# huggingface/distil-whisper

Hardware: AMD Instinct MI355X
Metric: training audio-seconds/s (distil-large-v3 student, 30 s clips) (higher is better)
Workload: dtype bf16

## Files before the change

### distil_whisper_amd/csrc/attention.hip

```cpp
#include "common.h"
#include "../../include/dwamd.h"

#define NEG_BIG (-1.0e30f)
#ifndef DW_ATTN_DEFER
#define DW_ATTN_DEFER 8
#endif
#ifndef DW_ATTN_IDLE_SKIP
#define DW_ATTN_IDLE_SKIP 1
#endif
typedef __attribute__((ext_vector_type(4))) unsigned u32x4;

struct AttnP {
    const bf16* q; const bf16* k; const bf16* v; bf16* o; float* lse;
    const bf16* d_o; float* delta; bf16* dq; bf16* dk; bf16* dv;
    long ldq, ldk, ldv, ldo, lddo, lddq, lddk, lddv;
    int B, H, Lq, Lk;
    long q_rows, kv_rows;
    float* dq_colsum;
    float* dv_colsum;
    const int* q_start; const int* q_len;
    const int* kv_start; const int* kv_len;
    int kv_B;
    int plain_order;
    float defer;
// ... 37 lines not shown
    char* const wr = patch + ln * 144 + hi * 8;
#pragma unroll
    for (int cb = 0; cb < 2; ++cb) {
        const f32x16& a = cb == 0 ? a0 : a1;
#pragma unroll
        for (int g = 0; g < 4; ++g) {
            bf16x4 w;
#pragma unroll
            for (int e = 0; e < 4; ++e) w[e] = f2bf(a[g * 4 + e] * mul);
            *(bf16x4*)(wr + cb * 64 + g * 16) = w;
        }
    }
    const int rr = lane >> 3, sc = lane & 7;
    u32x4 o[4];
#pragma unroll
    for (int it = 0; it < 4; ++it) o[it] = *(const u32x4*)(patch + (it * 8 + rr) * 144 + sc * 16);
    const unsigned loff = (unsigned)(rr * (int)ld + sc * 8) * 2u;
    char* const rb = (char*)(base + (long)row0 * ld);
#pragma unroll
    for (int it = 0; it < 4; ++it)
        if (row0 + it * 8 + rr < nrows) *(u32x4*)(rb + (long)it * 8 * ld * 2 + loff) = o[it];
}

__device__ __forceinline__ void colsum_t(float* colsum, bool ok, int cb, int hi, int ln, const f32x16& a, float mul) {
#pragma unroll
    for (int r = 0; r < 16; ++r) {
        float v = ok ? bf2f(f2bf(a[r] * mul)) : 0.f;
#pragma unroll
        for (int o = 1; o < 32; o <<= 1) v += __shfl_xor(v, o);
        if (ln == 0) atomicAdd(colsum + cb * 32 + (r & 3) + 8 * (r >> 2) + 4 * hi, v);
    }
}

__device__ __forceinline__ void attn_workgroup(int ntile, int H, bool plain, int& tile, int& h, int& b) {
    const int n = gridDim.x, L = blockIdx.x;
    const int xcd = L & 7, slot = L >> 3, q = n >> 3, r = n & 7;
    const int logical = plain ? L : xcd * q + min(xcd, r) + slot;
    tile = logical % ntile;
    const int bh = logical / ntile;
    h = bh % H;
    b = bh / H;
}

template <bool CAUSAL, int NW = 4, int ABL = 0, bool VL = false>
__global__ __launch_bounds__(64 * NW, CAUSAL ? 2 : 4) void attn_fwd_kernel(const AttnP p) {
    __shared__ __attribute__((aligned(1024))) char smem[2 * 16384];
    const int lane = threadIdx.x & 63;
    const int wave = __builtin_amdgcn_readfirstlane(threadIdx.x >> 6);
    const int hi = lane >> 5, ln = lane & 31;
    int tile, h, b;
    attn_workgroup((p.Lq + 32 * NW - 1) / (32 * NW), p.H, p.plain_order, tile, h, b);
    const int qb0 = tile * (32 * NW);
    long q_row0 = (long)b * p.q_rows, kv_row0 = (long)b * p.kv_rows;
    int Lq = p.Lq, Lk = p.Lk;
    if constexpr (VL) {
        q_row0 = p.q_start[b];
        Lq = p.q_len[b];
        if (p.kv_start) { kv_row0 = p.kv_start[b]; Lk = p.kv_len[b]; }
        else kv_row0 = (long)min(b, p.kv_B - 1) * p.kv_rows;
        if (qb0 >= Lq) return;
    }
    const int q = qb0 + wave * 32 + ln;
    const bool q_ok = q < Lq;
    const int qc = q_ok ? q : Lq - 1;
    const bf16* Q = p.q + q_row0 * p.ldq + h * 64;
    const bf16* K = p.k + kv_row0 * p.ldk + h * 64;
    const bf16* V = p.v + kv_row0 * p.ldv + h * 64;

    bf16x8 qf[4];
#pragma unroll
    for (int kk = 0; kk < 4; ++kk) qf[kk] = ldg8(Q, qc, p.ldq, kk * 16 + hi * 8);

    int nkt = (Lk + 63) >> 6;
    if (CAUSAL) {
        const int lim = ((min(qb0 + 32 * NW - 1, Lq - 1) + p.coff) >> 6) + 1;
        nkt = min(nkt, lim);
    }
    const float c = p.scale * 1.4426950408889634f;
    float m_run = NEG_BIG, l_run = 0.f;
    f32x16 o[2];
#pragma unroll
    for (int r = 0; r < 16; ++r) { o[0][r] = 0.f; o[1][r] = 0.f; }

    stage_tile64<NW>(K, p.ldk, 0, Lk, smem, wave, lane);
    stage_tile64<NW>(V, p.ldv, 0, Lk, smem + 8192, wave, lane);
    for (int kt = 0; kt < nkt; ++kt) {
        const int buf = kt & 1;
        if (!(ABL & 16) || kt == 0) {
            wait_vm0_seen();
            __syncthreads();
        }
        if (kt + 1 < nkt && !(ABL & 8)) {
            stage_tile64<NW>(K, p.ldk, (kt + 1) * 64, Lk, smem + (buf ^ 1) * 16384, wave, lane);
            stage_tile64<NW>(V, p.ldv, (kt + 1) * 64, Lk, smem + (buf ^ 1) * 16384 + 8192, wave, lane);
        }
        const char* tK = smem + buf * 16384;
        const char* tV = tK + 8192;
        if (DW_ATTN_IDLE_SKIP && qb0 + wave * 32 >= Lq) continue;
        f32x16 s[2];
#pragma unroll
        for (int kb = 0; kb < 2; ++kb) {
#pragma unroll
            for (int r = 0; r < 16; ++r) s[kb][r] = (ABL & 32) ? o[kb][r] : 0.f;
            if (!(ABL & 32)) {
#pragma unroll
                for (int kk = 0; kk < 4; ++kk)
                    s[kb] = __builtin_amdgcn_mfma_f32_32x32x16_bf16((ABL & 2) ? qf[kk ^ kb] : frag_rows(tK, kb, kk, lane), qf[kk], s[kb], 0, 0, 0);
            }
        }
        const int wq0 = qb0 + wave * 32 + (CAUSAL ? p.coff : 0);
        const bool need_mask = ((kt + 1) * 64 > Lk) || (CAUSAL && kt * 64 + 63 > wq0);
        if (CAUSAL && kt * 64 > wq0 + 31) continue;
        float mx = NEG_BIG;
        if (need_mask) {
#pragma unroll
            for (int kb = 0; kb < 2; ++kb)
#pragma unroll
                for (int r = 0; r < 16; ++r) {
                    const int key = kt * 64 + kb * 32 + (r & 3) + 8 * (r >> 2) + 4 * hi;
                    const bool ok = key < Lk && (!CAUSAL || key <= q + p.coff);
                    s[kb][r] = ok ? s[kb][r] : NEG_BIG;
                }
        }
#pragma unroll
        for (int kb = 0; kb < 2; ++kb)
#pragma unroll
            for (int r = 0; r < 16; ++r) mx = fmaxf(mx, s[kb][r]);
        mx = xhalf_max(mx);
        const bool move = __any((mx - m_run) * c > p.defer);
        const float m_new = move ? fmaxf(m_run, mx) : m_run;
        const float mc = m_new * c;
        f32x2 rs2[2] = {{0.f, 0.f}, {0.f, 0.f}};
        const f32x2 c2 = {c, c}, mc2 = {mc, mc};
#pragma unroll
        for (int kb = 0; kb < 2; ++kb)
#pragma unroll
            for (int r = 0; r < 16; r += 2) {
                f32x2 t = {s[kb][r], s[kb][r + 1]};
                t = t * c2 - mc2;
                f32x2 pv = {__builtin_amdgcn_exp2f(t[0]), __builtin_amdgcn_exp2f(t[1])};
                if (ABL & 1) pv = t;
                s[kb][r] = pv[0];
                s[kb][r + 1] = pv[1];
                rs2[(r >> 1) & 1] += pv;
            }
        rs2[0] += rs2[1];
        float rs = rs2[0][0] + rs2[0][1];
        rs = xhalf_sum(rs);
        if (move) {
            const float alpha = __builtin_amdgcn_exp2f((m_run - m_new) * c);
            l_run *= alpha;
#pragma unroll
            for (int r = 0; r < 16; ++r) { o[0][r] *= alpha; o[1][r] *= alpha; }
        }
        l_run += rs;
        m_run = m_new;
#pragma unroll
        for (int kb = 0; kb < 2; ++kb)
#pragma unroll
            for (int s2 = 0; s2 < 2; ++s2) {
                const bf16x8 pf = pack8(s[kb], s2);
                const int rb = kb * 32 + s2 * 16 + hi * 4;
                if (ABL & 64) {
                    o[kb][s2] += bf2f(pf[0]) + bf2f(pf[2]) + bf2f(pf[4]) + bf2f(pf[6]);
                    continue;
                }
#pragma unroll
                for (int db = 0; db < 2; ++db)
                    o[db] = __builtin_amdgcn_mfma_f32_32x32x16_bf16((ABL & 4) ? qf[db * 2 + s2] : frag_tr(tV, db, rb, rb + 8, lane), pf, o[db], 0, 0, 0);
            }
    }
    const float inv = 1.0f / l_run;
    bf16* O = p.o + q_row0 * p.ldo + h * 64;
    if (DW_ATTN_ROWSTORE && NW <= 7 && (p.ldo & 7) == 0 && ((uintptr_t)p.o & 15) == 0) {
        __syncthreads();
        store_rows(O, p.ldo, qb0 + wave * 32, Lq, smem + wave * 4608, lane, o[0], o[1], inv);
    } else {
        store_t(O, p.ldo, q, q_ok, 0, hi, o[0], inv);
        store_t(O, p.ldo, q, q_ok, 1, hi, o[1], inv);
    }
    if (!VL && p.lse && q_ok && hi == 0) p.lse[((long)b * p.H + h) * Lq + q] = m_run * p.scale + __logf(l_run);
}

template <int NW = 4, int OCC = 3>
__global__ __launch_bounds__(64 * NW, OCC) void attn_fwd_pipe_kernel(const AttnP p) {
    __shared__ __attribute__((aligned(1024))) char smem[3 * 16384];
    const int lane = threadIdx.x & 63;
    const int wave = __builtin_amdgcn_readfirstlane(threadIdx.x >> 6);
    const int hi = lane >> 5, ln = lane & 31;
    int tile, h, b;
    attn_workgroup((p.Lq + 32 * NW - 1) / (32 * NW), p.H, p.plain_order, tile, h, b);
    const int qb0 = tile * (32 * NW);
    const int q = qb0 + wave * 32 + ln;
    const bool q_ok = q < p.Lq;
    const int qc = q_ok ? q : p.Lq - 1;
    const bf16* Q = p.q + (long)b * p.q_rows * p.ldq + h * 64;
    const bf16* K = p.k + (long)b * p.kv_rows * p.ldk + h * 64;
    const bf16* V = p.v + (long)b * p.kv_rows * p.ldv + h * 64;
    bf16x8 qf[4];
#pragma unroll
    for (int kk = 0; kk < 4; ++kk) qf[kk] = ldg8(Q, qc, p.ldq, kk * 16 + hi * 8);
    const int nkt = (p.Lk + 63) >> 6;
    const float c = p.scale * 1.4426950408889634f;
    float m_run = NEG_BIG, l_run = 0.f;
    f32x16 o[2];
#pragma unroll
    for (int r = 0; r < 16; ++r) { o[0][r] = 0.f; o[1][r] = 0.f; }

    auto stage = [&](int kt, int st) __attribute__((always_inline)) {
        stage_tile64<NW>(K, p.ldk, kt * 64, p.Lk, smem + st * 16384, wave, lane);
        stage_tile64<NW>(V, p.ldv, kt * 64, p.Lk, smem + st * 16384 + 8192, wave, lane);
    };
    auto scores = [&](int kt, int st, f32x16 (&s)[2]) __attribute__((always_inline)) {
        const char* tK = smem + st * 16384;
#pragma unroll
        for (int kb = 0; kb < 2; ++kb) {
#pragma unroll
            for (int r = 0; r < 16; ++r) s[kb][r] = 0.f;
#pragma unroll
            for (int kk = 0; kk < 4; ++kk)
                s[kb] = __builtin_amdgcn_mfma_f32_32x32x16_bf16(frag_rows(tK, kb, kk, lane), qf[kk], s[kb], 0, 0, 0);
        }
        if ((kt + 1) * 64 > p.Lk) {
#pragma unroll
            for (int kb = 0; kb < 2; ++kb)
#pragma unroll
                for (int r = 0; r < 16; ++r) {
                    const int key = kt * 64 + kb * 32 + (r & 3) + 8 * (r >> 2) + 4 * hi;
                    s[kb][r] = key < p.Lk ? s[kb][r] : NEG_BIG;
                }
        }
    };
    auto softmax_pv = [&](int st, f32x16 (&s)[2]) __attribute__((always_inline)) {
        const char* tV = smem + st * 16384 + 8192;
        float mx = NEG_BIG;
#pragma unroll
        for (int kb = 0; kb < 2; ++kb)
#pragma unroll
            for (int r = 0; r < 16; ++r) mx = fmaxf(mx, s[kb][r]);
        mx = xhalf_max(mx);
        const bool move = __any((mx - m_run) * c > p.defer);
        const float m_new = move ? fmaxf(m_run, mx) : m_run;
        const float mc = m_new * c;
        f32x2 rs2[2] = {{0.f, 0.f}, {0.f, 0.f}};
        const f32x2 c2 = {c, c}, mc2 = {mc, mc};
#pragma unroll
        for (int kb = 0; kb < 2; ++kb)
#pragma unroll
            for (int r = 0; r < 16; r += 2) {
                f32x2 t = {s[kb][r], s[kb][r + 1]};
                t = t * c2 - mc2;
                const f32x2 pv = {__builtin_amdgcn_exp2f(t[0]), __builtin_amdgcn_exp2f(t[1])};
                s[kb][r] = pv[0];
                s[kb][r + 1] = pv[1];
                rs2[(r >> 1) & 1] += pv;
            }
        rs2[0] += rs2[1];
        float rs = rs2[0][0] + rs2[0][1];
        rs = xhalf_sum(rs);
        if (move) {
            const float alpha = __builtin_amdgcn_exp2f((m_run - m_new) * c);
            l_run *= alpha;
#pragma unroll
            for (int r = 0; r < 16; ++r) { o[0][r] *= alpha; o[1][r] *= alpha; }
        }
        l_run += rs;
        m_run = m_new;
#pragma unroll
        for (int kb = 0; kb < 2; ++kb)
#pragma unroll
            for (int s2 = 0; s2 < 2; ++s2) {
                const bf16x8 pf = pack8(s[kb], s2);
                const int rb = kb * 32 + s2 * 16 + hi * 4;
#pragma unroll
                for (int db = 0; db < 2; ++db)
                    o[db] = __builtin_amdgcn_mfma_f32_32x32x16_bf16(frag_tr(tV, db, rb, rb + 8, lane), pf, o[db], 0, 0, 0);
            }
    };

    stage(0, 0);
    if (nkt > 1) stage(1, 1);
    wait_vm0_seen();
    __syncthreads();
    f32x16 sa[2], sb[2];
    scores(0, 0, sa);
    auto iter = [&](int kt, int st0, int st1, int st2, f32x16 (&cur)[2], f32x16 (&nxt)[2]) __attribute__((always_inline)) {
        if (kt > 0) {
            wait_vm0_seen();
            __syncthreads();
        }
        if (kt + 2 < nkt) stage(kt + 2, st2);
        if (kt + 1 < nkt) scores(kt + 1, st1, nxt);
        softmax_pv(st0, cur);
    };
    int st0 = 0, st1 = 1, st2 = 2;
    for (int kt = 0; kt < nkt; kt += 2) {
        iter(kt, st0, st1, st2, sa, sb);
        if (kt + 1 < nkt) iter(kt + 1, st1, st2, st0, sb, sa);
        const int t0 = st0; st0 = st2; st2 = st1; st1 = t0;
    }
    const float inv = 1.0f / l_run;
    bf16* O = p.o + (long)b * p.q_rows * p.ldo + h * 64;
    if (DW_ATTN_ROWSTORE && (p.ldo & 7) == 0 && ((uintptr_t)p.o & 15) == 0) {
        __syncthreads();
        store_rows(O, p.ldo, qb0 + wave * 32, p.Lq, smem + wave * 4608, lane, o[0], o[1], inv);
    } else {
        store_t(O, p.ldo, q, q_ok, 0, hi, o[0], inv);
        store_t(O, p.ldo, q, q_ok, 1, hi, o[1], inv);
    }
    if (p.lse && q_ok && hi == 0) p.lse[((long)b * p.H + h) * p.Lq + q] = m_run * p.scale + __logf(l_run);
}

template <int NW, bool PRE>
__global__ __launch_bounds__(64 * NW) void attn_decode_kernel(const AttnP p) {
    extern __shared__ __attribute__((aligned(16))) float dsm[];
    const int lane = threadIdx.x & 63;
    const int wave = __builtin_amdgcn_readfirstlane(threadIdx.x >> 6);
    const int h = blockIdx.y, b = blockIdx.z;
    const int sub = lane >> 3, ds = (lane & 7) * 8;
    float* sc = dsm;
    float* part = dsm + ((p.Lk + 3) & ~3);
    float* redm = part + NW * 64;
    float* redl = redm + NW;
    const bf16* Q = p.q + (long)b * p.q_rows * p.ldq + h * 64 + ds;
    const bf16* K = p.k + (long)b * p.kv_rows * p.ldk + h * 64 + ds;
    const bf16* V = p.v + (long)b * p.kv_rows * p.ldv + h * 64 + ds;
    const float c = p.scale * 1.4426950408889634f;
    float qv[8];
    {
        const bf16x8 q8 = *(const bf16x8*)Q;
#pragma unroll
        for (int e = 0; e < 8; ++e) qv[e] = bf2f(q8[e]) * c;
    }
    constexpr int NIT = 12;
    bf16x8 kr[PRE ? NIT : 1], vr[PRE ? NIT : 1];
    if constexpr (PRE) {
#pragma unroll
        for (int it = 0; it < NIT; ++it) {
            int k = wave * 8 + it * (NW * 8) + sub;
            k = k < p.Lk ? k : p.Lk - 1;
            kr[it] = ld_stream<2>((const bf16x8*)(K + (long)k * p.ldk));
        }
#pragma unroll
        for (int it = 0; it < NIT; ++it) {
            int k = wave * 8 + it * (NW * 8) + sub;
            k = k < p.Lk ? k : p.Lk - 1;
            vr[it] = ld_stream<2>((const bf16x8*)(V + (long)k * p.ldv));
        }
    }
    float mx = NEG_BIG;
    float sreg[PRE ? NIT : 1];
    if constexpr (PRE) {
#pragma unroll
        for (int it = 0; it < NIT; ++it) {
            const int k = wave * 8 + it * (NW * 8) + sub;
            float s = 0.f;
#pragma unroll
            for (int e = 0; e < 8; ++e) s = fmaf(qv[e], bf2f(kr[it][e]), s);
            s += __shfl_xor(s, 1);
            s += __shfl_xor(s, 2);
            s += __shfl_xor(s, 4);
            sreg[it] = s;
            if (k < p.Lk) mx = fmaxf(mx, s);
        }
    } else {
    for (int k0 = wave * 8; k0 < p.Lk; k0 += NW * 8) {
        const int k = k0 + sub;
        float s = 0.f;
        if (k < p.Lk) {
            const bf16x8 k8 = *(const bf16x8*)(K + (long)k * p.ldk);
#pragma unroll
            for (int e = 0; e < 8; ++e) s = fmaf(qv[e], bf2f(k8[e]), s);
        }
        s += __shfl_xor(s, 1);
        s += __shfl_xor(s, 2);
        s += __shfl_xor(s, 4);
        if (k < p.Lk) {
            if ((lane & 7) == 0) sc[k] = s;
            mx = fmaxf(mx, s);
        }
    }
    }
    mx = wave_max(mx);
    if (lane == 0) redm[wave] = mx;
    __syncthreads();
    mx = redm[0];
#pragma unroll
    for (int i = 1; i < NW; ++i) mx = fmaxf(mx, redm[i]);
    float o[8] = {0.f, 0.f, 0.f, 0.f, 0.f, 0.f, 0.f, 0.f};
    float l = 0.f;
    if constexpr (PRE) {
#pragma unroll
        for (int it = 0; it < NIT; ++it) {
// ... 240 lines not shown
        const char* tG = tQ + 8192;
        const float* tL = (const float*)(tQ + 16384);
        const float* tD = tL + 64;
        const bool need_mask = MODE == 1 || (MODE == 2 && (((qt + 1) * 64 > p.Lq) || (wk0 + 31 >= p.Lk) || (CAUSAL && wk0 + 31 > qt * 64)));
        if (CAUSAL && wk0 > qt * 64 + 63) continue;
        if (DW_ATTN_IDLE_SKIP && wk0 >= p.Lk) continue;
#pragma unroll
        for (int qb = 0; qb < 2; ++qb) {
            f32x16 s, dp;
#pragma unroll
            for (int g = 0; g < 4; ++g) {
                const int ql = qb * 32 + g * 8 + hi * 4;
                const f32x4 l4 = *(const f32x4*)(tL + ql);
                const f32x4 d4 = *(const f32x4*)(tD + ql);
#pragma unroll
                for (int e = 0; e < 4; ++e) { s[g * 4 + e] = l4[e]; dp[g * 4 + e] = d4[e]; }
            }
#pragma unroll
            for (int kk = 0; kk < 4; ++kk) {
                s = __builtin_amdgcn_mfma_f32_32x32x16_bf16(frag_rows(tQ, qb, kk, lane), kf[kk], s, 0, 0, 0);
                dp = __builtin_amdgcn_mfma_f32_32x32x16_bf16(frag_rows(tG, qb, kk, lane), vf[kk], dp, 0, 0, 0);
            }
            f32x16 pr;
            const f32x2 c2 = {c, c};
#pragma unroll
            for (int r = 0; r < 16; r += 2) {
                f32x2 t = {s[r], s[r + 1]};
                t = t * c2;
                f32x2 pv = {__builtin_amdgcn_exp2f(t[0]), __builtin_amdgcn_exp2f(t[1])};
                if (need_mask) {
#pragma unroll
                    for (int e = 0; e < 2; ++e) {
                        const int qi = qt * 64 + qb * 32 + ((r + e) & 3) + 8 * ((r + e) >> 2) + 4 * hi_o;
                        pv[e] = (qi < p.Lq && k_ok_o && (!CAUSAL || key_o <= qi)) ? pv[e] : 0.f;
                    }
                }
                pr[r] = pv[0];
                pr[r + 1] = pv[1];
                const f32x2 d2 = {dp[r], dp[r + 1]};
                pv = pv * d2;
                s[r] = pv[0];
                s[r + 1] = pv[1];
            }
#pragma unroll
            for (int s2 = 0; s2 < 2; ++s2) {
                const bf16x8 pf = pack8(pr, s2);
                const bf16x8 df = pack8(s, s2);
                const int rb = qb * 32 + s2 * 16 + hi * 4;
#pragma unroll
                for (int db = 0; db < 2; ++db) {
                    av[db] = __builtin_amdgcn_mfma_f32_32x32x16_bf16(frag_tr(tG, db, rb, rb + 8, lane), pf, av[db], 0, 0, 0);
                    ak[db] = __builtin_amdgcn_mfma_f32_32x32x16_bf16(frag_tr(tQ, db, rb, rb + 8, lane), df, ak[db], 0, 0, 0);
                }
            }
        }
    }
    };
    if constexpr (CAUSAL) tiles(std::integral_constant<int, 2>{}, qt0, nqt);
    else {
        const int nfull = kb0 + 32 * NW - 1 >= p.Lk ? 0 : (p.Lq >> 6);
        tiles(std::integral_constant<int, 0>{}, 0, nfull);
        tiles(std::integral_constant<int, 1>{}, nfull, nqt);
    }
    bf16* DK = p.dk + (long)b * p.Lk * p.lddk + h * 64;
    bf16* DV = p.dv + (long)b * p.Lk * p.lddv + h * 64;
    if (DW_ATTN_ROWSTORE && NW <= 7 && ((p.lddk | p.lddv) & 7) == 0 && (((uintptr_t)p.dk | (uintptr_t)p.dv) & 15) == 0) {
        __syncthreads();
        store_rows(DK, p.lddk, kb0 + wave * 32, p.Lk, smem + wave * 4608, lane, ak[0], ak[1], p.scale);
        store_rows(DV, p.lddv, kb0 + wave * 32, p.Lk, smem + wave * 4608, lane, av[0], av[1], 1.0f);
    } else {
        store_t(DK, p.lddk, key, k_ok, 0, hi, ak[0], p.scale);
        store_t(DK, p.lddk, key, k_ok, 1, hi, ak[1], p.scale);
        store_t(DV, p.lddv, key, k_ok, 0, hi, av[0], 1.0f);
        store_t(DV, p.lddv, key, k_ok, 1, hi, av[1], 1.0f);
    }
    if (p.dv_colsum) {
        colsum_t(p.dv_colsum + ((long)b * p.H + h) * 64, k_ok, 0, hi, ln, av[0], 1.0f);
        colsum_t(p.dv_colsum + ((long)b * p.H + h) * 64, k_ok, 1, hi, ln, av[1], 1.0f);
    }
}

int g_attn_bwd_stage = 5;
int g_attn_bwd_waves = 4;
int g_attn_fwd_waves = 4;
int g_attn_fwd_pipe = 0;
int g_attn_plain_order = 0;
int g_attn_defer = DW_ATTN_DEFER;
int g_attn_ablate = 0;
int g_attn_decode = 1;
static int check_ld(int64_t ld) { return (ld & 7) ? DW_EINVAL : DW_OK; }

extern "C" int dw_attn_fwd_ex(const void* q, const void* k, const void* v, void* o, float* lse, int B, int H, int Lq,
                              int Lk, int64_t ldq, int64_t ldk, int64_t ldv, int64_t ldo, int64_t q_batch_rows,
                              int64_t kv_batch_rows, int causal, float scale, void* stream);

extern "C" int dw_attn_fwd(const void* q, const void* k, const void* v, void* o, float* lse, int B, int H, int Lq,
                           int Lk, int64_t ldq, int64_t ldk, int64_t ldv, int64_t ldo, int causal, float scale,
                           void* stream) {
    if (!lse) return DW_EINVAL;
    return dw_attn_fwd_ex(q, k, v, o, lse, B, H, Lq, Lk, ldq, ldk, ldv, ldo, Lq, Lk, causal, scale, stream);
}

extern "C" int dw_attn_fwd_ex(const void* q, const void* k, const void* v, void* o, float* lse, int B, int H, int Lq,
                              int Lk, int64_t ldq, int64_t ldk, int64_t ldv, int64_t ldo, int64_t q_batch_rows,
                              int64_t kv_batch_rows, int causal, float scale, void* stream) {
    DW_CLEAR_ERR();
    if (!q || !k || !v || !o || B <= 0 || H <= 0 || Lq <= 0 || Lk <= 0) return DW_EINVAL;
    if (q_batch_rows < Lq || kv_batch_rows < Lk) return DW_EINVAL;
    if ((int64_t)Lk * ldk >= (1LL << 31) || (int64_t)Lk * ldv >= (1LL << 31)) return DW_EINVAL;
    if (check_ld(ldq) || check_ld(ldk) || check_ld(ldv) || (ldo & 3)) return DW_EINVAL;
    if (((uintptr_t)q & 15) || ((uintptr_t)k & 15) || ((uintptr_t)v & 15) || ((uintptr_t)o & 7)) return DW_EINVAL;
    AttnP p = {};
    p.q = (const bf16*)q; p.k = (const bf16*)k; p.v = (const bf16*)v; p.o = (bf16*)o; p.lse = lse;
    p.ldq = ldq; p.ldk = ldk; p.ldv = ldv; p.ldo = ldo;
    p.B = B; p.H = H; p.Lq = Lq; p.Lk = Lk; p.scale = scale;
    p.q_rows = q_batch_rows; p.kv_rows = kv_batch_rows;
    if (causal != 0 && causal != 1 && causal != 2) return DW_EINVAL;
    if (causal == 2 && Lk < Lq) return DW_EINVAL;
    p.coff = causal == 2 ? Lk - Lq : 0;
    hipStream_t s = (hipStream_t)stream;
    if (Lq == 1 && g_attn_decode && Lk <= 8192) {
        const size_t smem = (((size_t)Lk + 3) & ~(size_t)3) * 4 + 16 * 64 * 4 + 2 * 16 * 4;
        if (Lk >= 512 && Lk <= 16 * 8 * 12 && (g_attn_decode & 2))
            hipLaunchKernelGGL((attn_decode_kernel<16, true>), dim3(1, H, B), dim3(1024), smem, s, p);
        else if (Lk >= 512) hipLaunchKernelGGL((attn_decode_kernel<16, false>), dim3(1, H, B), dim3(1024), smem, s, p);
        else hipLaunchKernelGGL((attn_decode_kernel<4, false>), dim3(1, H, B), dim3(256), smem, s, p);
        DW_CHECK_LAUNCH();
        return DW_OK;
    }
    const int g4 = (Lq + 127) / 128;
    dim3 grid(g4 * H * B), block(256);
    p.plain_order = g_attn_plain_order;
    p.defer = (float)g_attn_defer;
#ifdef DW_ABLATE
    if (!causal && g_attn_ablate) {
        switch (g_attn_ablate) {
#define ABLC(v) case v: hipLaunchKernelGGL((attn_fwd_kernel<false, 4, v>), grid, block, 0, s, p); break;
            ABLC(1) ABLC(2) ABLC(4) ABLC(6) ABLC(8) ABLC(24) ABLC(32) ABLC(64) ABLC(7) ABLC(31) ABLC(30)
#undef ABLC
            default: return DW_EINVAL;
        }
        return DW_OK;
    }
#endif
    const int g8 = (Lq + 255) / 256;
    if (causal) hipLaunchKernelGGL(attn_fwd_kernel<true>, grid, block, 0, s, p);
    else if (g_attn_fwd_pipe == 2 && Lk > 64) hipLaunchKernelGGL((attn_fwd_pipe_kernel<4, 2>), grid, block, 0, s, p);
    else if (g_attn_fwd_pipe && Lk > 64) hipLaunchKernelGGL((attn_fwd_pipe_kernel<4, 3>), grid, block, 0, s, p);
    else if (g_attn_fwd_waves == 8 && g8 * 2 == g4 && (long)g8 * H * B >= 512)
        hipLaunchKernelGGL((attn_fwd_kernel<false, 8>), dim3(g8 * H * B), dim3(512), 0, s, p);
    else hipLaunchKernelGGL(attn_fwd_kernel<false>, grid, block, 0, s, p);
    DW_CHECK_LAUNCH();
    return DW_OK;
}

extern "C" int dw_attn_fwd_varlen(const void* q, const void* k, const void* v, void* o, int n_seq, int H, int max_q, int Lk,
                                  int64_t ldq, int64_t ldk, int64_t ldv, int64_t ldo, const int32_t* q_start, const int32_t* q_len,
                                  const int32_t* kv_start, const int32_t* kv_len, int kv_batches, int64_t kv_batch_rows, int causal,
                                  float scale, void* stream) {
    DW_CLEAR_ERR();
    if (!q || !k || !v || !o || !q_start || !q_len || n_seq <= 0 || H <= 0 || max_q <= 0) return DW_EINVAL;
    if ((kv_start == nullptr) != (kv_len == nullptr)) return DW_EINVAL;
    if (!kv_start && (Lk <= 0 || kv_batches <= 0 || kv_batch_rows < Lk || causal)) return DW_EINVAL;
    if (causal != 0 && causal != 1) return DW_EINVAL;
    if (check_ld(ldq) || check_ld(ldk) || check_ld(ldv) || (ldo & 7)) return DW_EINVAL;
    if (((uintptr_t)q & 15) || ((uintptr_t)k & 15) || ((uintptr_t)v & 15) || ((uintptr_t)o & 15)) return DW_EINVAL;
    const int64_t lk_max = kv_start ? max_q : Lk;
    if (lk_max * ldk >= (1LL << 31) || lk_max * ldv >= (1LL << 31)) return DW_EINVAL;
    AttnP p = {};
    p.q = (const bf16*)q; p.k = (const bf16*)k; p.v = (const bf16*)v; p.o = (bf16*)o; p.lse = nullptr;
    p.ldq = ldq; p.ldk = ldk; p.ldv = ldv; p.ldo = ldo;
    p.B = n_seq; p.H = H; p.Lq = max_q; p.Lk = kv_start ? max_q : Lk; p.scale = scale;
    p.q_rows = 0; p.kv_rows = kv_batch_rows; p.coff = 0;
    p.q_start = q_start; p.q_len = q_len; p.kv_start = kv_start; p.kv_len = kv_len; p.kv_B = kv_batches;
    p.plain_order = g_attn_plain_order;
    p.defer = (float)g_attn_defer;
    hipStream_t s = (hipStream_t)stream;
    dim3 grid(((max_q + 127) / 128) * H * n_seq), block(256);
    if (causal) hipLaunchKernelGGL((attn_fwd_kernel<true, 4, 0, true>), grid, block, 0, s, p);
    else hipLaunchKernelGGL((attn_fwd_kernel<false, 4, 0, true>), grid, block, 0, s, p);
    DW_CHECK_LAUNCH();
    return DW_OK;
}

extern "C" int dw_attn_bwd_ex(const void* q, const void* k, const void* v, const void* o, const void* d_o,
                              const float* lse, float* delta, void* dq, void* dk, void* dv, int B, int H, int Lq, int Lk,
                              int64_t ldq, int64_t ldk, int64_t ldv, int64_t ldo, int64_t lddo, int64_t lddq,
                              int64_t lddk, int64_t lddv, int causal, float scale, float* dq_colsum, float* dv_colsum,
                              void* stream);
extern "C" int dw_attn_bwd(const void* q, const void* k, const void* v, const void* o, const void* d_o,
                           const float* lse, float* delta, void* dq, void* dk, void* dv, int B, int H, int Lq, int Lk,
                           int64_t ldq, int64_t ldk, int64_t ldv, int64_t ldo, int64_t lddo, int64_t lddq,
                           int64_t lddk, int64_t lddv, int causal, float scale, void* stream) {
    return dw_attn_bwd_ex(q, k, v, o, d_o, lse, delta, dq, dk, dv, B, H, Lq, Lk, ldq, ldk, ldv, ldo, lddo, lddq, lddk, lddv,
                          causal, scale, nullptr, nullptr, stream);
}

extern "C" int dw_attn_bwd_ex(const void* q, const void* k, const void* v, const void* o, const void* d_o,
                              const float* lse, float* delta, void* dq, void* dk, void* dv, int B, int H, int Lq, int Lk,
                              int64_t ldq, int64_t ldk, int64_t ldv, int64_t ldo, int64_t lddo, int64_t lddq,
                              int64_t lddk, int64_t lddv, int causal, float scale, float* dq_colsum, float* dv_colsum,
                              void* stream) {
    DW_CLEAR_ERR();
    if (!q || !k || !v || !o || !d_o || !lse || !delta || !dq || !dk || !dv) return DW_EINVAL;
    if (B <= 0 || H <= 0 || Lq <= 0 || Lk <= 0) return DW_EINVAL;
    if (causal != 0 && causal != 1) return DW_EINVAL;
    if (check_ld(ldq) || check_ld(ldk) || check_ld(ldv) || check_ld(ldo) || check_ld(lddo)) return DW_EINVAL;
    if ((lddq & 3) || (lddk & 3) || (lddv & 3)) return DW_EINVAL;
    if ((int64_t)Lk * ldk >= (1LL << 31) || (int64_t)Lk * ldv >= (1LL << 31) || (int64_t)Lq * ldq >= (1LL << 31) ||
        (int64_t)Lq * lddo >= (1LL << 31))
        return DW_EINVAL;
    if (((uintptr_t)q & 15) || ((uintptr_t)k & 15) || ((uintptr_t)v & 15) || ((uintptr_t)o & 15) ||
        ((uintptr_t)d_o & 15) || ((uintptr_t)dq & 7) || ((uintptr_t)dk & 7) || ((uintptr_t)dv & 7))
        return DW_EINVAL;
    AttnP p = {};
    p.q = (const bf16*)q; p.k = (const bf16*)k; p.v = (const bf16*)v; p.o = (bf16*)o; p.lse = (float*)lse;
    p.d_o = (const bf16*)d_o; p.delta = delta; p.dq = (bf16*)dq; p.dk = (bf16*)dk; p.dv = (bf16*)dv;
    p.ldq = ldq; p.ldk = ldk; p.ldv = ldv; p.ldo = ldo; p.lddo = lddo; p.lddq = lddq; p.lddk = lddk; p.lddv = lddv;
    p.B = B; p.H = H; p.Lq = Lq; p.Lk = Lk; p.scale = scale;
    p.dq_colsum = dq_colsum; p.dv_colsum = dv_colsum;
    hipStream_t s = (hipStream_t)stream;
    const int q4 = (Lq + 127) / 128, k4 = (Lk + 127) / 128;
    dim3 gq(q4 * H * B), gk(k4 * H * B), block(256);
    p.plain_order = g_attn_plain_order;
    p.defer = (float)g_attn_defer;
    const int fs = g_attn_bwd_stage;
    if (causal) {
        hipLaunchKernelGGL((attn_bwd_dq_kernel<true, false>), gq, block, 0, s, p);
        hipLaunchKernelGGL((attn_bwd_dkv_kernel<true, false, 2>), gk, block, 0, s, p);
    } else {
        const int q12 = (Lq + 383) / 384, k12 = (Lk + 383) / 384;
        const bool dq12 = g_attn_bwd_waves == 12 && q12 * 3 == q4 && (long)q12 * H * B >= 256;
        const bool dkv12 = g_attn_bwd_waves == 12 && k12 * 3 == k4 && (long)k12 * H * B >= 256;
        if (dq12) hipLaunchKernelGGL((attn_bwd_dq_kernel<false, true, 12>), dim3(q12 * H * B), dim3(768), 0, s, p);
// ... 12 lines not shown
```

### distil_whisper_amd/csrc/gemm.hip

```cpp
#include "gemm_common.h"
#include <mutex>
#include <unordered_map>

bool dw_gemm_skinny_ok(const GemmP& p, int trans_a, int trans_b);
int dw_gemm_skinny_launch(const GemmP& p, hipStream_t s);
int dw_gemm_tile256_launch(const GemmP& p, int ta, int tb, hipStream_t s);
int dw_gemm_tile128_launch(const GemmP& p, int ta, int tb, hipStream_t s);
int dw_gemm_wp8_nn_launch(const GemmP& p, hipStream_t s);
int dw_gemm_wp8_nt_launch(const GemmP& p, hipStream_t s);
int dw_gemm_wp8_nn320_launch(const GemmP& p, hipStream_t s);
int dw_gemm_wp8_nt320_launch(const GemmP& p, hipStream_t s);
int dw_gemm_wp8_nn128_launch(const GemmP& p, hipStream_t s);
int dw_gemm_wp8_nt128_launch(const GemmP& p, hipStream_t s);
int dw_gemm_wp16_nn_launch(const GemmP& p, hipStream_t s);
int dw_gemm_wp16_tt_launch(const GemmP& p, hipStream_t s);
int dw_gemm_wp16_nn_small_launch(const GemmP& p, hipStream_t s);
int dw_gemm_wp16_nt_small_launch(const GemmP& p, hipStream_t s);

extern int g_attn_bwd_stage;
extern int g_attn_decode;
extern int g_attn_ablate;
extern int g_attn_fwd_waves;
extern int g_attn_fwd_pipe;
extern int g_attn_plain_order;
extern int g_attn_defer;
extern int g_attn_bwd_waves;
extern int g_logmel_mfma;
extern int g_decode_fuse_off;
extern int g_skinny_wide;
extern int g_ln_variant;
enum { GEMM_RULE = 0,
       GEMM_REFERENCE = 1,
       GEMM_FORCE_320 = 2 };
static int g_gemm_mode = GEMM_RULE;
int g_gemm_strip = 0;
int g_gemm_cus = 256;
static int g_gemm_stage_next = 1;
static int g_gemm_dynamic = 1;
static int g_gemm_small_m = 1;
static int g_gemm_row_tail = 1;

static int* gemm_sched_slot(hipStream_t s) {
    static std::mutex mu;
    static std::unordered_map<hipStream_t, int*> slots;
    std::lock_guard<std::mutex> lock(mu);
    auto it = slots.find(s);
    if (it != slots.end()) return it->second;
    hipStreamCaptureStatus st = hipStreamCaptureStatusNone;
    if (hipStreamIsCapturing(s, &st) != hipSuccess || st != hipStreamCaptureStatusNone) { (void)hipGetLastError(); return nullptr; }
    int* ptr = nullptr;
    if (hipMalloc((void**)&ptr, 64) != hipSuccess || hipMemsetAsync(ptr, 0, 64, s) != hipSuccess) { (void)hipGetLastError(); return nullptr; }
    slots[s] = ptr;
    return ptr;
}
int g_gemm_strip_budget = 4;
extern "C" int dw_debug_set(int key, int value) {
    if (key == 0) { if (value < GEMM_RULE || value > GEMM_FORCE_320) return DW_EINVAL; g_gemm_mode = value; return DW_OK; }
    if (key == 1) { g_gemm_strip = value; return DW_OK; }
    if (key == 3) { g_attn_bwd_stage = value; return DW_OK; }
    if (key == 4) { g_attn_decode = value; return DW_OK; }
    if (key == 5) { g_logmel_mfma = value; return DW_OK; }
    if (key == 6) { g_gemm_strip_budget = value; return DW_OK; }
    if (key == 7) { g_decode_fuse_off = value; return DW_OK; }
    if (key == 8) { g_skinny_wide = value; return DW_OK; }
    if (key == 10) { g_gemm_dynamic = value; return DW_OK; }
    if (key == 11) { g_gemm_stage_next = value; return DW_OK; }
    if (key == 17) { g_attn_bwd_waves = value; return DW_OK; }
    if (key == 21) { g_ln_variant = value; return DW_OK; }
    if (key == 22) { g_gemm_row_tail = value; return DW_OK; }
    if (key == 25) { if (value < 0 || value > 1) return DW_EINVAL; g_gemm_small_m = value; return DW_OK; }
    if (key == 26) { g_attn_fwd_pipe = value; return DW_OK; }
    if (key == 18) { g_attn_plain_order = value; return DW_OK; }
    if (key == 23) { if (value < 0 || value > 64) return DW_EINVAL; g_attn_defer = value; return DW_OK; }
    if (key == 16) { g_attn_fwd_waves = value; return DW_OK; }
    if (key == 15) { g_attn_ablate = value; return DW_OK; }
    if (key == 9) { if (value < 8 || value > 256 || (value & 7)) return DW_EINVAL; g_gemm_cus = value; return DW_OK; }
    return DW_EINVAL;
}

__global__ __launch_bounds__(256) void reduce_slices_kernel(const float* part, long stride, int slices, float* out,
                                                            long n, int accumulate) {
    const long i = ((long)blockIdx.x * 256 + threadIdx.x) * 4;
    if (i >= n) return;
    f32x4 acc = accumulate ? *(const f32x4*)(out + i) : f32x4{0.f, 0.f, 0.f, 0.f};
    for (int s = 0; s < slices; ++s) {
        const f32x4 v = *(const f32x4*)(part + s * stride + i);
#pragma unroll
        for (int e = 0; e < 4; ++e) acc[e] += v[e];
    }
    *(f32x4*)(out + i) = acc;
}

extern "C" int dw_reduce_slices(const float* part, int64_t stride, int slices, float* out, int64_t n, int accumulate,
                                void* stream) {
    DW_CLEAR_ERR();
    if (!part || !out || slices < 1 || n <= 0 || (n & 3) || (stride & 3) || ((uintptr_t)part & 15) ||
        ((uintptr_t)out & 15))
        return DW_EINVAL;
    hipLaunchKernelGGL(reduce_slices_kernel, dim3((n / 4 + 255) / 256), dim3(256), 0, (hipStream_t)stream, part,
                       (long)stride, slices, out, (long)n, accumulate);
    DW_CHECK_LAUNCH();
    return DW_OK;
}

__global__ __launch_bounds__(256) void reduce_slices_ld_kernel(const float* part, long slice_stride, long ld_part, int slices,
                                                               float* out, long ld_out, int rows, int cols4, int accumulate) {
    const long i = (long)blockIdx.x * 256 + threadIdx.x;
    if (i >= (long)rows * cols4) return;
    const int r = (int)(i / cols4), c = (int)(i - (long)r * cols4) * 4;
    float* o = out + (long)r * ld_out + c;
    f32x4 acc = accumulate ? *(const f32x4*)o : f32x4{0.f, 0.f, 0.f, 0.f};
    const float* src = part + (long)r * ld_part + c;
    for (int s = 0; s < slices; ++s) {
        const f32x4 v = *(const f32x4*)(src + s * slice_stride);
#pragma unroll
        for (int e = 0; e < 4; ++e) acc[e] += v[e];
    }
    *(f32x4*)o = acc;
}
extern "C" int dw_reduce_slices_ld(const float* part, int64_t slice_stride, int64_t ld_part, int slices, float* out, int64_t ld_out,
                                   int rows, int cols, int accumulate, void* stream) {
    DW_CLEAR_ERR();
    if (!part || !out || slices < 1 || rows <= 0 || cols <= 0 || (cols & 3) || (ld_part & 3) || (ld_out & 3) || (slice_stride & 3) ||
        ld_part < cols || ld_out < cols || ((uintptr_t)part & 15) || ((uintptr_t)out & 15))
        return DW_EINVAL;
    const long n = (long)rows * (cols / 4);
    hipLaunchKernelGGL(reduce_slices_ld_kernel, dim3((n + 255) / 256), dim3(256), 0, (hipStream_t)stream, part, (long)slice_stride,
                       (long)ld_part, slices, out, (long)ld_out, rows, cols / 4, accumulate);
    DW_CHECK_LAUNCH();
    return DW_OK;
}

enum GemmKernel {
    K_SKINNY,
    K_TILE128,
    K_TILE256,
    K_WP8_M128,
    K_WP16_SMALL,
    K_WP8_320,
    K_WP16_NN,
    K_WP8_NN,
    K_WP8_NT,
    K_WP16_TT,
};

static GemmKernel gemm_choose(const DwGemm* g, const GemmP& p) {
    const bool ta = g->trans_a, tb = g->trans_b, nn = !ta && !tb;
    const bool one_slice = p.split_k == 1 && !p.atomic;
    const bool ref = g_gemm_mode == GEMM_REFERENCE;
    const bool res_f32 = g->r && g->r_dtype == DW_F32 && g->c_dtype == DW_F32;
    const long cus = g_gemm_cus, tn = (g->n + 255) / 256;
    const long t256 = (long)((g->m + 255) / 256) * tn;
    const bool fits320 = !ta && one_slice && g->m % 320 == 0 && g->n % 256 == 0;
    int tile = g->tile;
    if ((tile == 0 || tile == 16) && dw_gemm_skinny_ok(p, ta, tb)) return K_SKINNY;
    bool one_round_320 = false, small_m_256 = false;
    if (tile != 128 && tile != 256) {
// ... 125 lines not shown
```

Before: 2803.

## Add 64-query-per-wave attention forward kernel reusing K/V fragments

Adds a non-causal attention forward kernel in which each wave handles 64 query rows (two 32-row blocks) instead of 32. K and V fragments are loaded from shared memory once per tile and reused for both query blocks, which halves LDS reads per unit of MFMA work. Tail-tile masking is split out through a compile-time flag so full tiles skip the mask check. The old pipelined kernel and the 8-wave variants are removed, and the new kernel becomes the default. Register pressure rises (two accumulator sets, Q fragments and cached K/V fragments) and occupancy is capped at 2, so fewer workgroups run per CU.

```diff
diff --git a/distil_whisper_amd/csrc/attention.hip b/distil_whisper_amd/csrc/attention.hip
--- a/distil_whisper_amd/csrc/attention.hip
+++ b/distil_whisper_amd/csrc/attention.hip
@@ -143,8 +143,8 @@
 #pragma unroll
     for (int r = 0; r < 16; ++r) { o[0][r] = 0.f; o[1][r] = 0.f; }
 
-    stage_tile64<NW>(K, p.ldk, 0, Lk, smem, wave, lane);
-    stage_tile64<NW>(V, p.ldv, 0, Lk, smem + 8192, wave, lane);
+    stage_tile64<4>(K, p.ldk, 0, Lk, smem, wave, lane);
+    stage_tile64<4>(V, p.ldv, 0, Lk, smem + 8192, wave, lane);
     for (int kt = 0; kt < nkt; ++kt) {
         const int buf = kt & 1;
         if (!(ABL & 16) || kt == 0) {
@@ -152,8 +152,8 @@
             __syncthreads();
         }
         if (kt + 1 < nkt && !(ABL & 8)) {
-            stage_tile64<NW>(K, p.ldk, (kt + 1) * 64, Lk, smem + (buf ^ 1) * 16384, wave, lane);
-            stage_tile64<NW>(V, p.ldv, (kt + 1) * 64, Lk, smem + (buf ^ 1) * 16384 + 8192, wave, lane);
+            stage_tile64<4>(K, p.ldk, (kt + 1) * 64, Lk, smem + (buf ^ 1) * 16384, wave, lane);
+            stage_tile64<4>(V, p.ldv, (kt + 1) * 64, Lk, smem + (buf ^ 1) * 16384 + 8192, wave, lane);
         }
         const char* tK = smem + buf * 16384;
         const char* tV = tK + 8192;
@@ -243,57 +243,46 @@
     if (!VL && p.lse && q_ok && hi == 0) p.lse[((long)b * p.H + h) * Lq + q] = m_run * p.scale + __logf(l_run);
 }
 
-template <int NW = 4, int OCC = 3>
-__global__ __launch_bounds__(64 * NW, OCC) void attn_fwd_pipe_kernel(const AttnP p) {
-    __shared__ __attribute__((aligned(1024))) char smem[3 * 16384];
+__global__ __launch_bounds__(256, 2) void attn_fwd_w64_kernel(const AttnP p) {
+    __shared__ __attribute__((aligned(1024))) char smem[2 * 16384];
     const int lane = threadIdx.x & 63;
     const int wave = __builtin_amdgcn_readfirstlane(threadIdx.x >> 6);
     const int hi = lane >> 5, ln = lane & 31;
     int tile, h, b;
-    attn_workgroup((p.Lq + 32 * NW - 1) / (32 * NW), p.H, p.plain_order, tile, h, b);
-    const int qb0 = tile * (32 * NW);
-    const int q = qb0 + wave * 32 + ln;
-    const bool q_ok = q < p.Lq;
-    const int qc = q_ok ? q : p.Lq - 1;
-    const bf16* Q = p.q + (long)b * p.q_rows * p.ldq + h * 64;
-    const bf16* K = p.k + (long)b * p.kv_rows * p.ldk + h * 64;
-    const bf16* V = p.v + (long)b * p.kv_rows * p.ldv + h * 64;
-    bf16x8 qf[4];
-#pragma unroll
-    for (int kk = 0; kk < 4; ++kk) qf[kk] = ldg8(Q, qc, p.ldq, kk * 16 + hi * 8);
-    const int nkt = (p.Lk + 63) >> 6;
+    attn_workgroup((p.Lq + 255) / 256, p.H, p.plain_order, tile, h, b);
+    const int qb0 = tile * 256;
+    const int Lq = p.Lq, Lk = p.Lk;
+    const long q_row0 = (long)b * p.q_rows, kv_row0 = (long)b * p.kv_rows;
+    const int wq0 = qb0 + wave * 64;
+    const bf16* Q = p.q + q_row0 * p.ldq + h * 64;
+    const bf16* K = p.k + kv_row0 * p.ldk + h * 64;
+    const bf16* V = p.v + kv_row0 * p.ldv + h * 64;
+
+    bf16x8 qf[2][4];
+#pragma unroll
+    for (int j = 0; j < 2; ++j) {
+        const int q = wq0 + j * 32 + ln;
+        const int qc = q < Lq ? q : Lq - 1;
+#pragma unroll
+        for (int kk = 0; kk < 4; ++kk) qf[j][kk] = ldg8(Q, qc, p.ldq, kk * 16 + hi * 8);
+    }
+    const int nkt = (Lk + 63) >> 6;
     const float c = p.scale * 1.4426950408889634f;
-    float m_run = NEG_BIG, l_run = 0.f;
-    f32x16 o[2];
-#pragma unroll
-    for (int r = 0; r < 16; ++r) { o[0][r] = 0.f; o[1][r] = 0.f; }
-
-    auto stage = [&](int kt, int st) __attribute__((always_inline)) {
-        stage_tile64<NW>(K, p.ldk, kt * 64, p.Lk, smem + st * 16384, wave, lane);
-        stage_tile64<NW>(V, p.ldv, kt * 64, p.Lk, smem + st * 16384 + 8192, wave, lane);
-    };
-    auto scores = [&](int kt, int st, f32x16 (&s)[2]) __attribute__((always_inline)) {
-        const char* tK = smem + st * 16384;
-#pragma unroll
-        for (int kb = 0; kb < 2; ++kb) {
-#pragma unroll
-            for (int r = 0; r < 16; ++r) s[kb][r] = 0.f;
-#pragma unroll
-            for (int kk = 0; kk < 4; ++kk)
-                s[kb] = __builtin_amdgcn_mfma_f32_32x32x16_bf16(frag_rows(tK, kb, kk, lane), qf[kk], s[kb], 0, 0, 0);
-        }
-        if ((kt + 1) * 64 > p.Lk) {
+    float m_run[2] = {NEG_BIG, NEG_BIG}, l_run[2] = {0.f, 0.f};
+    f32x16 o[2][2];
+#pragma unroll
+    for (int r = 0; r < 16; ++r) { o[0][0][r] = 0.f; o[0][1][r] = 0.f; o[1][0][r] = 0.f; o[1][1][r] = 0.f; }
+
+    auto softmax = [&](auto maskc, int kt, f32x16 (&s)[2], float& m_run, float& l_run, f32x16 (&o)[2]) __attribute__((always_inline)) {
+        if constexpr (decltype(maskc)::value) {
 #pragma unroll
             for (int kb = 0; kb < 2; ++kb)
 #pragma unroll
                 for (int r = 0; r < 16; ++r) {
                     const int key = kt * 64 + kb * 32 + (r & 3) + 8 * (r >> 2) + 4 * hi;
-                    s[kb][r] = key < p.Lk ? s[kb][r] : NEG_BIG;
+                    s[kb][r] = key < Lk ? s[kb][r] : NEG_BIG;
                 }
         }
-    };
-    auto softmax_pv = [&](int st, f32x16 (&s)[2]) __attribute__((always_inline)) {
-        const char* tV = smem + st * 16384 + 8192;
         float mx = NEG_BIG;
 #pragma unroll
         for (int kb = 0; kb < 2; ++kb)
@@ -327,49 +316,88 @@
         }
         l_run += rs;
         m_run = m_new;
+    };
+    auto pv_mfma = [&](const f32x16 (&s)[2], f32x16 (&o)[2], const bf16x8 (&vf)[2][2][2]) __attribute__((always_inline)) {
 #pragma unroll
         for (int kb = 0; kb < 2; ++kb)
 #pragma unroll
             for (int s2 = 0; s2 < 2; ++s2) {
                 const bf16x8 pf = pack8(s[kb], s2);
-                const int rb = kb * 32 + s2 * 16 + hi * 4;
-#pragma unroll
-                for (int db = 0; db < 2; ++db)
-                    o[db] = __builtin_amdgcn_mfma_f32_32x32x16_bf16(frag_tr(tV, db, rb, rb + 8, lane), pf, o[db], 0, 0, 0);
+#pragma unroll
+                for (int db = 0; db < 2; ++db) o[db] = __builtin_amdgcn_mfma_f32_32x32x16_bf16(vf[kb][s2][db], pf, o[db], 0, 0, 0);
             }
     };
 
-    stage(0, 0);
-    if (nkt > 1) stage(1, 1);
-    wait_vm0_seen();
-    __syncthreads();
-    f32x16 sa[2], sb[2];
-    scores(0, 0, sa);
-    auto iter = [&](int kt, int st0, int st1, int st2, f32x16 (&cur)[2], f32x16 (&nxt)[2]) __attribute__((always_inline)) {
-        if (kt > 0) {
+    stage_tile64<4>(K, p.ldk, 0, Lk, smem, wave, lane);
+    stage_tile64<4>(V, p.ldv, 0, Lk, smem + 8192, wave, lane);
+    auto tiles = [&](auto maskc, int kt_begin, int kt_end) __attribute__((always_inline)) {
+        for (int kt = kt_begin; kt < kt_end; ++kt) {
+            const int buf = kt & 1;
             wait_vm0_seen();
             __syncthreads();
-        }
-        if (kt + 2 < nkt) stage(kt + 2, st2);
-        if (kt + 1 < nkt) scores(kt + 1, st1, nxt);
-        softmax_pv(st0, cur);
+            if (kt + 1 < nkt) {
+                stage_tile64<4>(K, p.ldk, (kt + 1) * 64, Lk, smem + (buf ^ 1) * 16384, wave, lane);
+                stage_tile64<4>(V, p.ldv, (kt + 1) * 64, Lk, smem + (buf ^ 1) * 16384 + 8192, wave, lane);
+            }
+            const char* tK = smem + buf * 16384;
+            const char* tV = tK + 8192;
+            if (DW_ATTN_IDLE_SKIP && wq0 >= Lq) continue;
+            bf16x8 kf[2][4];
+#pragma unroll
+            for (int kb = 0; kb < 2; ++kb)
+#pragma unroll
+                for (int kk = 0; kk < 4; ++kk) kf[kb][kk] = frag_rows(tK, kb, kk, lane);
+            f32x16 s[2][2];
+#pragma unroll
+            for (int j = 0; j < 2; ++j)
+#pragma unroll
+                for (int kb = 0; kb < 2; ++kb) {
+#pragma unroll
+                    for (int r = 0; r < 16; ++r) s[j][kb][r] = 0.f;
+#pragma unroll
+                    for (int kk = 0; kk < 4; ++kk) s[j][kb] = __builtin_amdgcn_mfma_f32_32x32x16_bf16(kf[kb][kk], qf[j][kk], s[j][kb], 0, 0, 0);
+                }
+            bf16x8 vf[2][2][2];
+#pragma unroll
+            for (int kb = 0; kb < 2; ++kb)
+#pragma unroll
+                for (int s2 = 0; s2 < 2; ++s2) {
+                    const int rb = kb * 32 + s2 * 16 + hi * 4;
+#pragma unroll
+                    for (int db = 0; db < 2; ++db) vf[kb][s2][db] = frag_tr(tV, db, rb, rb + 8, lane);
+                }
+            softmax(maskc, kt, s[0], m_run[0], l_run[0], o[0]);
+            pv_mfma(s[0], o[0], vf);
+            softmax(maskc, kt, s[1], m_run[1], l_run[1], o[1]);
+            pv_mfma(s[1], o[1], vf);
+        }
     };
-    int st0 = 0, st1 = 1, st2 = 2;
-    for (int kt = 0; kt < nkt; kt += 2) {
-        iter(kt, st0, st1, st2, sa, sb);
-        if (kt + 1 < nkt) iter(kt + 1, st1, st2, st0, sb, sa);
-        const int t0 = st0; st0 = st2; st2 = st1; st1 = t0;
-    }
-    const float inv = 1.0f / l_run;
-    bf16* O = p.o + (long)b * p.q_rows * p.ldo + h * 64;
+    const int nfull = Lk >> 6;
+    tiles(std::false_type{}, 0, nfull);
+    tiles(std::true_type{}, nfull, nkt);
+
+    bf16* O = p.o + q_row0 * p.ldo + h * 64;
     if (DW_ATTN_ROWSTORE && (p.ldo & 7) == 0 && ((uintptr_t)p.o & 15) == 0) {
         __syncthreads();
-        store_rows(O, p.ldo, qb0 + wave * 32, p.Lq, smem + wave * 4608, lane, o[0], o[1], inv);
+#pragma unroll
+        for (int j = 0; j < 2; ++j)
+            store_rows(O, p.ldo, wq0 + j * 32, Lq, smem + wave * 4608, lane, o[j][0], o[j][1], 1.0f / l_run[j]);
     } else {
-        store_t(O, p.ldo, q, q_ok, 0, hi, o[0], inv);
-        store_t(O, p.ldo, q, q_ok, 1, hi, o[1], inv);
-    }
-    if (p.lse && q_ok && hi == 0) p.lse[((long)b * p.H + h) * p.Lq + q] = m_run * p.scale + __logf(l_run);
+#pragma unroll
+        for (int j = 0; j < 2; ++j) {
+            const int q = wq0 + j * 32 + ln;
+            const float inv = 1.0f / l_run[j];
+            store_t(O, p.ldo, q, q < Lq, 0, hi, o[j][0], inv);
+            store_t(O, p.ldo, q, q < Lq, 1, hi, o[j][1], inv);
+        }
+    }
+    if (p.lse && hi == 0) {
+#pragma unroll
+        for (int j = 0; j < 2; ++j) {
+            const int q = wq0 + j * 32 + ln;
+            if (q < Lq) p.lse[((long)b * p.H + h) * Lq + q] = m_run[j] * p.scale + __logf(l_run[j]);
+        }
+    }
 }
 
 template <int NW, bool PRE>
@@ -776,8 +804,7 @@
 
 int g_attn_bwd_stage = 5;
 int g_attn_bwd_waves = 4;
-int g_attn_fwd_waves = 4;
-int g_attn_fwd_pipe = 0;
+int g_attn_fwd_ref = 0;
 int g_attn_plain_order = 0;
 int g_attn_defer = DW_ATTN_DEFER;
 int g_attn_ablate = 0;
@@ -837,13 +864,9 @@
         return DW_OK;
     }
 #endif
-    const int g8 = (Lq + 255) / 256;
     if (causal) hipLaunchKernelGGL(attn_fwd_kernel<true>, grid, block, 0, s, p);
-    else if (g_attn_fwd_pipe == 2 && Lk > 64) hipLaunchKernelGGL((attn_fwd_pipe_kernel<4, 2>), grid, block, 0, s, p);
-    else if (g_attn_fwd_pipe && Lk > 64) hipLaunchKernelGGL((attn_fwd_pipe_kernel<4, 3>), grid, block, 0, s, p);
-    else if (g_attn_fwd_waves == 8 && g8 * 2 == g4 && (long)g8 * H * B >= 512)
-        hipLaunchKernelGGL((attn_fwd_kernel<false, 8>), dim3(g8 * H * B), dim3(512), 0, s, p);
-    else hipLaunchKernelGGL(attn_fwd_kernel<false>, grid, block, 0, s, p);
+    else if (g_attn_fwd_ref) hipLaunchKernelGGL(attn_fwd_kernel<false>, grid, block, 0, s, p);
+    else hipLaunchKernelGGL(attn_fwd_w64_kernel, dim3(((Lq + 255) / 256) * H * B), block, 0, s, p);
     DW_CHECK_LAUNCH();
     return DW_OK;
 }
diff --git a/distil_whisper_amd/csrc/gemm.hip b/distil_whisper_amd/csrc/gemm.hip
--- a/distil_whisper_amd/csrc/gemm.hip
+++ b/distil_whisper_amd/csrc/gemm.hip
@@ -20,8 +20,7 @@
 extern int g_attn_bwd_stage;
 extern int g_attn_decode;
 extern int g_attn_ablate;
-extern int g_attn_fwd_waves;
-extern int g_attn_fwd_pipe;
+extern int g_attn_fwd_ref;
 extern int g_attn_plain_order;
 extern int g_attn_defer;
 extern int g_attn_bwd_waves;
@@ -69,10 +68,9 @@
     if (key == 21) { g_ln_variant = value; return DW_OK; }
     if (key == 22) { g_gemm_row_tail = value; return DW_OK; }
     if (key == 25) { if (value < 0 || value > 1) return DW_EINVAL; g_gemm_small_m = value; return DW_OK; }
-    if (key == 26) { g_attn_fwd_pipe = value; return DW_OK; }
+    if (key == 27) { if (value < 0 || value > 1) return DW_EINVAL; g_attn_fwd_ref = value; return DW_OK; }
     if (key == 18) { g_attn_plain_order = value; return DW_OK; }
     if (key == 23) { if (value < 0 || value > 64) return DW_EINVAL; g_attn_defer = value; return DW_OK; }
-    if (key == 16) { g_attn_fwd_waves = value; return DW_OK; }
     if (key == 15) { g_attn_ablate = value; return DW_OK; }
     if (key == 9) { if (value < 8 || value > 256 || (value & 7)) return DW_EINVAL; g_gemm_cus = value; return DW_OK; }
     return DW_EINVAL;
```

Result: no change. 2809, median of 6 (+0.2%).
